# KanaLab/mesh

Measured on AMD Instinct MI355X. Metric: closest-point queries/sec vs 1M-face mesh at 1/2/4/8 MI355X + HBM GB/s, higher is better.
Workload: dtype f64; 1 GPU; C3: geodesic icosphere freq 224 (1003520 faces, 501762 vertices), 100000000 uniform queries in [-1.1,1.1]^3 (seed 3) per step, sharded contiguously over the GPUs; faces=1003520, queries_total=100000000, queries_per_gpu=100000000

## Files before the change

### mesh_amd/csrc/nearest.hip

```cpp
#include <algorithm>
#include <cstdlib>
#include <cstring>
#include <mutex>
#include <vector>
#include <type_traits>

#include "internal.h"


namespace msh {

struct DeferRec {
    uint32_t slot;
    uint32_t face;
    int32_t leaf;
    uint32_t roff;
    double best;
    uint32_t rcnt;
    uint32_t sbound;
};
static_assert(sizeof(DeferRec) == 32, "DeferRec must be 32 B");

#ifndef MSH_P2_SPLIT
#define MSH_P2_SPLIT 8
#endif
#ifndef MSH_P2_HEAVY
#define MSH_P2_HEAVY 0.97
#endif
constexpr unsigned kP2Split = MSH_P2_SPLIT;
constexpr double kP2Heavy = MSH_P2_HEAVY;
constexpr unsigned kP2SplitItems = 1u << 16;
constexpr uint32_t kP2Whole = 0xFFFFFFFFu;
struct P2Cand {
    double best;
    uint32_t face;
    int32_t leaf;
};

struct KnnArgs {
    const BNode* nodes;
    const void* leaves;
    size_t T;
    const double* q;
    const double* n;
    const uint32_t* perm;
    const uint32_t* qperm;
    uint32_t* inv_w;
    size_t S;
    QRes* res;
    double* res_w;
    uint32_t* out_face;
    uint32_t* out_part;
    double* out_pt;
    double* out_dist;
    double* out_w;
    double eps;
    double org[3];
    double tm;
    const double* orgs;
    size_t qper;
    size_t npm;
    size_t root0;
    unsigned* counters;
    unsigned ntiles;
    uint2* spill;
    int spill_depth;
    unsigned long long* stats;
    unsigned budget;
    int phase;
    bool direct;
    bool rec_leaf;
    bool list;
    const uint32_t* cut;
    int cut_wide;
    int cut_G;
    double cut_lo[3], cut_iw[3];
    size_t nunits;
    DeferRec* deferred;
    unsigned* n_deferred;
    unsigned max_deferred;
    uint2* resume;
    unsigned* n_resume;
    unsigned resume_cap;
// ... 151 lines not shown
            --sp;
            const Ent e = stack_get(lds, spill, sp);
            if (E::bound(e) <= pol.limf) {
                node = E::ref(e);
                return true;
            }
        }
        return false;
    }
    template <class Pol, bool STATS>
    __device__ inline bool step(const BNode* __restrict__ nodes, const QF& qf, Pol& pol, Ent* __restrict__ lds,
                                uint2* __restrict__ spill, unsigned& n_nodes, unsigned& n_leaves) {
        const NodeV nd = load_node(nodes, node);
        if (STATS) ++n_nodes;
        float d0, d1;
        node_child_bounds(nd, qf, d0, d1);
        const int c0 = nd.child(0), c1 = nd.child(1);
        bool h0 = d0 <= pol.limf, h1 = d1 <= pol.limf;
        if (h0 && c0 < 0) {
            pol.test(~c0);
            if (STATS) ++n_leaves;
            h0 = false;
        }
        if (h1 && c1 < 0) {
            pol.test(~c1);
            if (STATS) ++n_leaves;
            h1 = false;
        }
        h0 = h0 && d0 <= pol.limf;
        h1 = h1 && d1 <= pol.limf;
        if (h0 && h1) {
            int nearc = c0, farc = c1;
            float dfar = d1;
            if (d1 < d0) { nearc = c1; farc = c0; dfar = d0; }
            push((unsigned)farc, __float_as_uint(dfar), lds, spill);
            node = nearc;
            return true;
        }
        if (h0) { node = c0; return true; }
        if (h1) { node = c1; return true; }
        return pop(pol, lds, spill);
    }
    template <class Pol, bool STATS, bool PF = false>
    __device__ inline bool step_collect(const BNode* __restrict__ nodes, const QF& qf, const Pol& pol,
                                        Ent* __restrict__ lds, uint2* __restrict__ spill, unsigned& n_nodes, int& p0,
                                        int& p1, int room = 2, const float4* nb = nullptr, uint32_t wsl = 0) {
        bool more = false;
        if (node < 0) {
            p0 = ~node;
        } else {
            const NodeV nd = PF ? node_from_lds(nb) : load_node(nodes, node);
            if (STATS) ++n_nodes;
            float d0, d1;
            node_child_bounds(nd, qf, d0, d1);
            const int c0 = nd.child(0), c1 = nd.child(1);
            const float lim = pol.limf;
            const bool h0 = d0 <= lim, h1 = d1 <= lim;
            const bool l0 = h0 && c0 < 0, l1 = h1 && c1 < 0;
            const bool i0 = h0 && c0 >= 0, i1 = h1 && c1 >= 0;
            const bool first1 = d1 < d0;
            if (l0 && l1) {
                if (room < 2) {
                    p0 = first1 ? ~c1 : ~c0;
                    node = first1 ? c0 : c1;
                    more = true;
                } else {
                    p0 = ~c0;
                    p1 = ~c1;
                }
            } else {
                if (l0) p0 = ~c0;
                if (l1) p0 = ~c1;
                if (i0 && i1) push((unsigned)(first1 ? c0 : c1), __float_as_uint(first1 ? d0 : d1), lds, spill);
                if (i0 || i1) {
                    node = (i0 && i1) ? (first1 ? c1 : c0) : (i0 ? c0 : c1);
                    more = true;
                }
            }
        }
        const bool r = more || pop(pol, lds, spill);
        if (PF && r && node >= 0) node_prefetch(nodes, node, wsl);
        return r;
    }
};
typedef WalkerT<Ent8> Walker;

__device__ inline D3 heidrich_bary(const D3& p, const D3& a, const D3& b, const D3& c) {
    const D3 u = vsub(b, a), v = vsub(c, a);
    const D3 n = vcross(u, v);
    double s = n.x * n.x + n.y * n.y + n.z * n.z;
    if (s == 0.0) s = 2.220446049250313e-16;
    const double inv = 1.0 / s;
    const D3 w = vsub(p, a);
    const double b2 = vdot(vcross(u, w), n) * inv;
    const double b1 = vdot(vcross(w, v), n) * inv;
    return D3{1.0 - b1 - b2, b1, b2};
}

template <int MODE, class Pol>
__device__ inline void write_result(const KnnArgs& a, size_t i, const D3& q, const Pol& pol) {
    const bool rec = a.res && (!a.direct || a.phase == 1 || a.phase == 3 || a.phase == 4);
    const bool out = !a.res || a.direct;
    const size_t r = a.res ? (size_t)a.perm[i] : i;
    if constexpr (MODE == 2) {
        const double dist = pol.best_leaf >= 0 ? sqrt(pol.best) : NAN;
        if (rec) store_qres(a.res + i, pol.best_face, 0u, dist, 0.0, 0.0);
        if (out) {
            a.out_face[r] = pol.best_face;
            a.out_dist[r] = dist;
        }
        return;
    }
    const TriRec* tris = static_cast<const TriRec*>(a.leaves);
    D3 ta, tb, tc, o = D3{NAN, NAN, NAN}, w = D3{NAN, NAN, NAN};
    uint32_t face = MSH_NO_FACE;
    int part = 0;
    if (pol.best_leaf >= 0) {
        load_tri(tris, pol.best_leaf, ta, tb, tc, face);
        closest_on_triangle(q, ta, tb, tc, o, part);
        if (MODE == 3) w = heidrich_bary(o, ta, tb, tc);
    }
    if (rec) {
        store_qres(a.res + i, face, a.rec_leaf ? (uint32_t)pol.best_leaf : (uint32_t)part, o.x, o.y, o.z);
        if (MODE == 3 && !a.direct) {
            a.res_w[3 * i] = w.x;
            a.res_w[3 * i + 1] = w.y;
            a.res_w[3 * i + 2] = w.z;
        }
    }
    if (!out) return;
    a.out_face[r] = face;
    if (MODE == 0 && a.out_part) a.out_part[r] = (uint32_t)part;
    a.out_pt[3 * r] = o.x;
    a.out_pt[3 * r + 1] = o.y;
    a.out_pt[3 * r + 2] = o.z;
    if (MODE == 3) {
        a.out_w[3 * r] = w.x;
        a.out_w[3 * r + 1] = w.y;
        a.out_w[3 * r + 2] = w.z;
    }
}

template <int MODE>
struct PolOf { using T = TriPol; };
template <>
struct PolOf<1> { using T = NrmPol; };
template <>
struct PolOf<2> { using T = PtPol; };

template <int MODE>
__device__ inline typename PolOf<MODE>::T make_pol(const KnnArgs& a, size_t i, const D3& q) {
    typename PolOf<MODE>::T pol;
    if constexpr (MODE == 2) {
        pol.pts = static_cast<const PtRec*>(a.leaves);
    } else {
        pol.tris = static_cast<const TriRec*>(a.leaves);
    }
    pol.q = q;
    if constexpr (MODE == 1) {
        pol.qn = D3{a.n[3 * i], a.n[3 * i + 1], a.n[3 * i + 2]};
        const double nq = sqrt(vdot(pol.qn, pol.qn));
        pol.eps = a.eps;
        pol.pmin = fmin(a.eps * (1 - nq), a.eps * (1 + nq));
    }
    pol.best = INFINITY;
    pol.shared = INFINITY;
    pol.best_face = MSH_NO_FACE;
    pol.best_leaf = -1;
    pol.limf = INFINITY;
    return pol;
}


__device__ inline D3 load_q(const KnnArgs& a, size_t i) {
    const size_t r = a.qperm ? (size_t)a.qperm[i] : i;
    return D3{a.q[3 * r], a.q[3 * r + 1], a.q[3 * r + 2]};
}

#ifndef MSH_KLEAD
#define MSH_KLEAD 8
#endif
#ifndef MSH_KFWIN
#define MSH_KFWIN 64
#endif
#ifndef MSH_FOLLOW_CELL
#define MSH_FOLLOW_CELL 0
#endif
#ifndef MSH_RESUME
#define MSH_RESUME 1
#endif
constexpr unsigned kLead = MSH_KLEAD;
constexpr unsigned kLead2 = 256;
constexpr size_t kFWin = MSH_KFWIN;
constexpr size_t kLWin = 8;
static_assert(kLead2 % kLead == 0 && kLead2 / kLead >= 2, "kLead2: a multiple of kLead");
constexpr int kLeafQ = 4;
constexpr int kLeafRound = 2;

__device__ inline size_t slot_of(const KnnArgs& a, size_t k) {
    if (a.phase == 3) return k * kLead2;
    if (a.phase == 4) return k * kLead;
    if (a.phase == 1) {
        constexpr size_t r = kLead2 / kLead;
        return kLead * (k + k / (r - 1) + 1);
    }
    if (a.phase == 2) {
        const size_t g = k / (kLead - 1);
        return g * kLead + (k - g * (kLead - 1)) + 1;
    }
    return k;
}

__device__ inline int leader_leaf(const KnnArgs& a, size_t i, const D3& q, size_t window, size_t stride) {
    const size_t base = (i / window) * window;
    const size_t mesh = a.orgs ? i / a.qper : 0;
    double h = INFINITY;
    int leaf = -1;
    for (size_t L = 0; L < window; L += stride) {
        const size_t li = base + L;
        if (li >= a.S) break;
        if (a.orgs && li / a.qper != mesh) continue;
        const uint4 r0 = reinterpret_cast<const uint4*>(a.res + li)[0];
        if (r0.x == MSH_NO_FACE) continue;
        const double2 r1 = reinterpret_cast<const double2*>(a.res + li)[1];
        const double x = __longlong_as_double((long long)(((unsigned long long)r0.w << 32) | r0.z));
        const double dx = q.x - x, dy = q.y - r1.x, dz = q.z - r1.y;
        const double d2 = dx * dx + dy * dy + dz * dz;
        if (d2 < h) {
            h = d2;
            leaf = (int)r0.y;
        }
    }
    return leaf;
}

__device__ inline unsigned lanes_below(unsigned long long m) {
    return __builtin_amdgcn_mbcnt_hi((unsigned)(m >> 32), __builtin_amdgcn_mbcnt_lo((unsigned)m, 0u));
}

#ifndef MSH_KPEND
#define MSH_KPEND 32
#endif
constexpr int kPend = MSH_KPEND;
#ifndef MSH_TILE_PF
#define MSH_TILE_PF 1
#endif

constexpr unsigned kRing = 256;
constexpr size_t kListMaxLeaves = (size_t)1 << 26;
constexpr size_t kLeadMinLeaves = 4096;

#ifndef MSH_KNN_WAVES
#define MSH_KNN_WAVES 4
#endif
#define MSH_KNN_ATTR __attribute__((amdgpu_waves_per_eu(MODE == 1 ? 1 : MSH_KNN_WAVES)))
constexpr size_t kNoCell = ~(size_t)0;
__device__ inline size_t cut_cell(const KnnArgs& a, const D3& q) {
    if (!a.cut) return kNoCell;
    const double G = (double)a.cut_G;
    const double ux = (q.x - a.cut_lo[0]) * a.cut_iw[0], uy = (q.y - a.cut_lo[1]) * a.cut_iw[1],
                 uz = (q.z - a.cut_lo[2]) * a.cut_iw[2];
    if (!(ux >= 0.0 && ux < G && uy >= 0.0 && uy < G && uz >= 0.0 && uz < G)) return kNoCell;
    return ((size_t)(unsigned)uz * (size_t)a.cut_G + (unsigned)uy) * (size_t)a.cut_G + (unsigned)ux;
}
__device__ inline const uint32_t* cut_rec(const KnnArgs& a, size_t cell) {
    return a.cut + cell * (a.cut_wide ? 16 : 8);
}
template <class Pol, class W>
__device__ inline bool cut_start(const KnnArgs& a, size_t cell, const Pol& pol, W& w, typename W::Ent* __restrict__ lds,
                                 uint2* __restrict__ spill) {
    const uint32_t* r = cut_rec(a, cell);
    if (a.cut_wide) {
        const uint4* c = reinterpret_cast<const uint4*>(r);
        uint4 e[4];
#pragma unroll
        for (int j = 0; j < 4; ++j) e[j] = c[j];
        auto put = [&](uint32_t ref, uint32_t sb) {
            if (ref != kCutEmpty) w.push(ref, sb, lds, spill);
        };
#pragma unroll
        for (int j = 3; j >= 1; --j) {
            put(e[j].z, e[j].w);
            put(e[j].x, e[j].y);
        }
        put(e[0].z, e[0].w);
    } else {
        const uint4* c = reinterpret_cast<const uint4*>(r);
        const uint4 e0 = c[0], e1 = c[1];
        const uint32_t e[kCutK] = {e0.y, e0.z, e0.w, e1.x, e1.y, e1.z, e1.w};
#pragma unroll
        for (int j = kCutK - 1; j >= 0; --j)
            if ((int)e[j] >= 0) w.push((uint32_t)Ent4::ref(e[j]), e[j] & 0xFFE00000u, lds, spill);
    }
    return w.pop(pol, lds, spill);
}

template <int MODE, bool STATS, bool LIST, bool PF>
__global__ __launch_bounds__(kBlock) MSH_KNN_ATTR void k_knn(KnnArgs a) {
    constexpr bool kCompact = MODE == 0 || MODE == 3;
    constexpr bool kList = (MODE == 0 || MODE == 3) && LIST;
    constexpr bool kPF = kList && PF;
    typedef typename std::conditional<kPF, Ent4, Ent8>::type E;
    __shared__ typename E::T stk[kStack * kBlock];
    __shared__ float4 nbuf[kPF ? 4 * kBlock : 1];
    constexpr size_t kEntWords = kCompact && !kList ? (size_t)kBlock * kLeafQ * 2 : 1;
    constexpr size_t kListWords = kList ? 4 * (kRing + 64 * 4) : 1;
    __shared__ uint32_t lsh[kEntWords > kListWords ? kEntWords : kListWords];
    uint2* lent = reinterpret_cast<uint2*>(lsh);
    const int tid = threadIdx.x, lane = tid & 63;
    typename E::T* lds = stk + tid;
    const int wv_u = __builtin_amdgcn_readfirstlane(tid >> 6);
    const uint32_t wsl = (uint32_t)(size_t)(__attribute__((address_space(3))) float4*)(nbuf + (kPF ? wv_u * 256 : 0));
    const float4* nb = nbuf + (kPF ? (tid >> 6) * 256 + lane : 0);
    uint2* ent = lent + (kCompact ? (tid >> 6) * 64 * kLeafQ : 0);
    uint2* spill = a.spill ? a.spill + (size_t)blockIdx.x * kBlock * (size_t)a.spill_depth + tid : nullptr;
    const unsigned group = blockIdx.x & 7u;
    unsigned long long u_trav_it = 0, u_trav_lanes = 0, u_leaf_it = 0, u_leaf_lanes = 0;
    unsigned n_nodes = 0, n_leaves = 0;
    unsigned n_impr = 0, n_hinted = 0, n_hint_won = 0;
#if MSH_TILE_PF
    const unsigned glo = (unsigned)(((unsigned long long)a.ntiles * group) >> 3);
    const unsigned ghi = (unsigned)(((unsigned long long)a.ntiles * (group + 1)) >> 3);
    unsigned nxt = ~0u;
#endif
    for (;;) {
        unsigned tile = 0;
#if MSH_TILE_PF
        if (lane == 0) tile = (nxt != ~0u && glo + nxt < ghi) ? glo + nxt : dequeue_tile(a.counters, a.ntiles, group);
#else
        if (lane == 0) tile = dequeue_tile(a.counters, a.ntiles, group);
#endif
        tile = __shfl(tile, 0);
        if (tile >= a.ntiles) break;
        const size_t k = (size_t)tile * 64 + lane;
        size_t i = 0;
        bool live = k < a.nunits;
        if (live) {
            i = slot_of(a, k);
            live = i < a.S;
        }
        const D3 q = live ? load_q(a, i) : D3{0.0, 0.0, 0.0};
#if MSH_TILE_PF
        if (lane == 0) nxt = glo < ghi ? atomicAdd(&a.counters[group * 32], 1u) : ~0u;
#endif
        if (live && a.inv_w && !a.direct) a.inv_w[a.qperm[i]] = (uint32_t)i;
        auto pol = make_pol<MODE>(a, i, q);
        const bool fin = live && finite3(q);
        if (live && !fin) {
            if (!STATS || a.res) write_result<MODE>(a, i, q, pol);
        }
        int hint_leaf = -1;
        const size_t cell = kList && fin ? cut_cell(a, q) : kNoCell;
        if constexpr (MODE == 0 || MODE == 3) {
            if (kList && a.cut && cell != kNoCell && a.phase != 2) {
                const int lf = (int)cut_rec(a, cell)[0];
                if (STATS) hint_leaf = lf;
                if (lf >= 0) {
                    pol.test(lf);
                    if (STATS) {
                        ++n_leaves;
                        ++n_hinted;
                    }
                }
            } else if (fin && (a.phase == 2 || a.phase == 1)) {
                const int lf = a.phase == 2 ? leader_leaf(a, i, q, kFWin, kLead) : leader_leaf(a, i, q, kLWin * kLead2, kLead2);
                if (STATS) hint_leaf = lf;
#if MSH_FOLLOW_CELL
                const int lc = (kList && a.cut && cell != kNoCell) ? (int)cut_rec(a, cell)[0] : -1;
#pragma nounroll
                for (int j = 0; j < 2; ++j) {
                    const int h = j == 0 ? lf : (lc != lf ? lc : -1);
                    if (h >= 0) {
                        pol.test(h);
                        if (STATS) ++n_leaves;
                    }
                }
                if (STATS && lf >= 0) ++n_hinted;
#else
                if (lf >= 0) {
                    pol.test(lf);
                    if (STATS) {
                        ++n_leaves;
                        ++n_hinted;
                    }
                }
#endif
            }
        }
        if (a.T == 1) {
            if (fin) {
                pol.test(0);
                if (STATS) ++n_leaves;
                if (!STATS || a.res) write_result<MODE>(a, i, q, pol);
            }
            continue;
        }
        if constexpr (kList) {
          {
            QF qf;
            const int root = query_root(a, i, q, qf);
            WalkerT<E> w{root, 0};
            bool start = fin;
            if (cell != kNoCell) start = cut_start(a, cell, pol, w, lds, spill);
            if (kPF && start && w.node >= 0) node_prefetch(a.nodes, w.node, wsl);
            uint32_t* ring = lsh + (tid >> 6) * (kRing + 64 * 4);
            unsigned long long* bd = reinterpret_cast<unsigned long long*>(ring + kRing);
            unsigned long long* bfl = bd + 64;
            bool active = start, want_defer = false, deferred = false;
            int nq = 0;
            unsigned last_pos = 0;
            unsigned head = 0, tail = 0;
            unsigned steps = 0;
            const unsigned max_steps = (unsigned)min(a.T, (size_t)UINT_MAX);
            unsigned tot = 0;
            auto run_rounds = [&](unsigned upto) {
                while (head != upto) {
                    const unsigned n = min(64u, upto - head);
                    bd[lane] = (unsigned long long)__double_as_longlong(pol.best);
                    bfl[lane] = ~0ull;
                    const bool valid = (unsigned)lane < n;
                    const uint32_t en = ring[(head + (valid ? (unsigned)lane : 0u)) & (kRing - 1)];
                    const int src = (int)(en & 63u);
                    const int leaf = (int)(en >> 6);
                    const D3 x = D3{__shfl(pol.q.x, src), __shfl(pol.q.y, src), __shfl(pol.q.z, src)};
                    uint32_t f;
                    const double d2 = pol.eval(leaf, x, f);
                    const unsigned long long kb = (unsigned long long)__double_as_longlong(d2);
                    asm volatile("" ::: "memory");
                    if (valid) atomicMin(&bd[src], kb);
                    asm volatile("" ::: "memory");
                    if (valid && bd[src] == kb) atomicMin(&bfl[src], ((unsigned long long)f << 32) | (unsigned)leaf);
                    asm volatile("" ::: "memory");
                    const unsigned long long nb = bd[lane], nf = bfl[lane];
                    const double nd = __longlong_as_double((long long)nb);
                    const uint32_t nface = (uint32_t)(nf >> 32);
                    if (nf != ~0ull && (nd < pol.best || (nd == pol.best && nface < pol.best_face))) {
                        pol.best = nd;
                        pol.best_face = nface;
                        pol.best_leaf = (int)(uint32_t)nf;
                        pol.relim();
                        if (STATS) ++n_impr;
                    }
                    asm volatile("" ::: "memory");
                    if (STATS) {
                        if (valid) ++n_leaves;
                        if (lane == 0) {
                            ++u_leaf_it;
                            u_leaf_lanes += n;
                        }
                    }
                    head += n;
                }
                if ((int)(last_pos - head) < 0) nq = 0;
            };
            unsigned dslot = 0;
            for (;;) {
                if (want_defer && nq == 0) {
                    want_defer = false;
                    dslot = atomicAdd(a.n_deferred, 1u);
                    if (dslot < a.max_deferred) {
                        active = false;
                        deferred = true;
                    }
                }
                const bool can = active && !want_defer && nq < kPend;
                const bool any = __ballot(can) != 0ull;
                if (!any && tail == head) break;
                if (STATS) {
                    const int nt = __popcll(__ballot(can));
                    if (lane == 0 && any) {
                        ++u_trav_it;
                        u_trav_lanes += nt;
                    }
                }
                int l0 = -1, l1 = -1;
                if (can) {
                    active = w.template step_collect<decltype(pol), STATS, kPF>(a.nodes, qf, pol, lds, spill, n_nodes,
                                                                                  l0, l1, kPend - nq, nb, wsl);
                    ++steps;
                    if (STATS) ++tot;
                    if (active && steps >= max_steps) active = false;
                    if (active && steps == a.budget) want_defer = true;
                }
                if (l0 < 0) {
                    l0 = l1;
                    l1 = -1;
                }
                const unsigned long long m1 = __ballot(l0 >= 0), m2 = __ballot(l1 >= 0);
                const unsigned pos = tail + lanes_below(m1) + lanes_below(m2);
                if (l0 >= 0) {
                    ring[pos & (kRing - 1)] = ((uint32_t)l0 << 6) | (uint32_t)lane;
                    last_pos = pos;
                    ++nq;
                }
                if (l1 >= 0) {
                    ring[(pos + 1) & (kRing - 1)] = ((uint32_t)l1 << 6) | (uint32_t)lane;
                    last_pos = pos + 1;
                    ++nq;
                }
                tail += (unsigned)(__popcll(m1) + __popcll(m2));
                const unsigned upto = any ? head + ((tail - head) & ~63u) : tail;
                if (upto != head) run_rounds(upto);
            }
            if (deferred) {
                if ((a.phase == 1 || a.phase == 3 || a.phase == 4) && a.res) {
                    D3 o = D3{NAN, NAN, NAN};
                    uint32_t f = MSH_NO_FACE;
                    if (pol.best_leaf >= 0) {
                        D3 ta, tb, tc;
                        int part;
                        load_tri(static_cast<const TriRec*>(a.leaves), pol.best_leaf, ta, tb, tc, f);
                        closest_on_triangle(q, ta, tb, tc, o, part);
                    }
                    store_qres(a.res + i, f, (uint32_t)pol.best_leaf, o.x, o.y, o.z);
                }
                DeferRec r;
                r.slot = (uint32_t)i;
                r.face = pol.best_face;
                r.leaf = pol.best_leaf;
                r.roff = 0;
                r.best = pol.best;
                r.rcnt = 0;
                r.sbound = 0x7F800000u;
                if (a.max_best) atomicMax(a.max_best, (unsigned long long)__double_as_longlong(pol.best));
                if (a.resume) {
                    const unsigned cnt = (unsigned)w.sp + 1;
                    const unsigned off = atomicAdd(a.n_resume, cnt);
                    if (off + cnt <= a.resume_cap) {
                        uint2* dst = a.resume + off;
                        for (int j = 0; j < w.sp; ++j) {
                            const typename E::T e = stack_get(lds, spill, j);
                            dst[j] = make_uint2((uint32_t)E::ref(e), __float_as_uint(E::bound(e)));
                        }
                        dst[w.sp] = make_uint2((uint32_t)w.node, 0u);
                        r.roff = off;
                        r.rcnt = cnt;
                    }
                }
                a.deferred[dslot] = r;
            }
            if (STATS) {
                unsigned mx = tot, sm = tot;
                for (int o = 32; o > 0; o >>= 1) {
                    mx = max(mx, (unsigned)__shfl_xor((int)mx, o));
                    sm += (unsigned)__shfl_xor((int)sm, o);
                }
                unsigned long long* h = a.stats + 8 + 9 * (a.phase == 3 ? 0 : ((a.phase == 1 || a.phase == 4) ? 1 : 2));
                if (lane == 0) {
                    atomicAdd(h + 0, 1ull);
                    atomicAdd(h + 1, (unsigned long long)mx);
                    atomicAdd(h + 2, (unsigned long long)sm);
                    atomicAdd(h + 3, (unsigned long long)min(mx, 128u));
                    atomicAdd(h + 4, (unsigned long long)min(mx, 256u));
                    atomicAdd(h + 5, (unsigned long long)min(mx, 512u));
                }
                if (tot > 128) atomicAdd(h + 6, 1ull);
                if (tot > 256) atomicAdd(h + 7, 1ull);
                if (tot > 512) atomicAdd(h + 8, 1ull);
            }
            if (STATS && fin && hint_leaf >= 0 && pol.best_leaf == hint_leaf) ++n_hint_won;
            if (deferred) continue;
            if (fin && (!STATS || a.res)) write_result<MODE>(a, i, q, pol);
            continue;
          }
        }
        if constexpr (!kList) {
        {
            QF qf;
            const int root = query_root(a, i, q, qf);
            Walker w{root, 0};
            bool active = fin, deferred = false;
            int q0 = -1, q1 = -1, q2 = -1, q3 = -1, nq = 0;
            auto enqueue = [&](int x) {
                if (x < 0) return;
                if (kLeafQ > 3) q3 = q2;
                q2 = q1;
                q1 = q0;
                q0 = x;
                ++nq;
            };
            auto test_queue = [&](int most) {
                const int n = min(nq, most);
#pragma nounroll
                for (int k = 0; k < n; ++k) {
                    pol.test(q0);
                    q0 = q1;
                    q1 = q2;
                    if (kLeafQ > 3) q2 = q3;
                }
                nq -= n;
            };
            unsigned steps = 0;
            const unsigned max_steps = (unsigned)min(a.T, (size_t)UINT_MAX);
            unsigned tot = 0;
            for (;;) {
                const bool can = active && nq <= kLeafQ - 1;
                const bool has = nq > 0;
                const unsigned long long bl = __ballot(has);
                const unsigned long long bt = __ballot(can);
                if ((bl | bt) == 0ull) break;
                const bool flush = bt == 0ull || __ballot(has && !can) != 0ull;
                if (bl != 0ull && flush) {
                    if constexpr (kCompact) {
                        const unsigned long long lt = (1ull << lane) - 1ull;
                        const unsigned long long m1 = bl, m2 = __ballot(nq >= 2), m3 = __ballot(nq >= 3),
                                                 m4 = kLeafQ > 3 ? __ballot(nq >= 4) : 0ull;
                        const int pos = __popcll(m1 & lt) + __popcll(m2 & lt) + __popcll(m3 & lt) + __popcll(m4 & lt);
                        const int E = __popcll(m1) + __popcll(m2) + __popcll(m3) + __popcll(m4);
                        if (nq >= 1) ent[pos] = make_uint2((unsigned)q0, (unsigned)lane);
                        if (nq >= 2) ent[pos + 1] = make_uint2((unsigned)q1, (unsigned)lane);
                        if (nq >= 3) ent[pos + 2] = make_uint2((unsigned)q2, (unsigned)lane);
                        if (kLeafQ > 3 && nq >= 4) ent[pos + 3] = make_uint2((unsigned)q3, (unsigned)lane);
                        asm volatile("" ::: "memory");
                        bool better = false;
                        for (int base = 0; base < E; base += 64) {
                            const uint2 en = ent[min(base + lane, E - 1)];
                            const int src = (int)en.y;
                            const D3 x = D3{__shfl(pol.q.x, src), __shfl(pol.q.y, src), __shfl(pol.q.z, src)};
                            uint32_t f;
                            const double d2 = pol.eval((int)en.x, x, f);
                            if (STATS && base + lane < E) ++n_leaves;
#pragma unroll
                            for (int e = 0; e < kLeafQ; ++e) {
                                const int at = pos + e - base;
                                const bool mine = e < nq && at >= 0 && at < 64;
                                const int from = mine ? at : lane;
                                const double dk = __shfl(d2, from);
                                const uint32_t fk = (uint32_t)__shfl((int)f, from);
                                if (mine) {
                                    const bool b = pol.offer(dk, fk, e == 0 ? q0 : (e == 1 ? q1 : (e == 2 ? q2 : q3)));
                                    better |= b;
                                    if (STATS && b) ++n_impr;
                                }
                            }
                        }
                        asm volatile("" ::: "memory");
                        if (better) pol.relim();
                        if (STATS && lane == 0) {
                            u_leaf_it += (unsigned long long)((E + 63) / 64);
                            u_leaf_lanes += (unsigned long long)E;
                        }
                        nq = 0;
                    } else {
                        if (STATS && lane == 0) {
                            ++u_leaf_it;
// ... 365 lines not shown
__global__ __launch_bounds__(kBlock) void k_unpermute(const QRes* __restrict__ res, const double* __restrict__ w, int nw,
                                                      const uint32_t* __restrict__ inv, size_t S, SlotOut o) {
    const size_t j = (size_t)blockIdx.x * kBlock + threadIdx.x;
    if (j >= S) return;
    const size_t i = inv[j];
    const uint4 r0 = reinterpret_cast<const uint4*>(res + i)[0];
    const double2 r1 = reinterpret_cast<const double2*>(res + i)[1];
    const double x = __longlong_as_double((long long)(((unsigned long long)r0.w << 32) | r0.z));
    if (o.face) o.face[j] = r0.x;
    if (o.part) o.part[j] = r0.y;
    if (o.dist) o.dist[j] = x;
    if (o.pt) {
        o.pt[3 * j] = x;
        o.pt[3 * j + 1] = r1.x;
        o.pt[3 * j + 2] = r1.y;
    }
    for (int k = 0; k < nw; ++k) o.w[(size_t)nw * j + k] = w[(size_t)nw * i + k];
}

int unpermute_results(const QRes* d_res, const double* d_w, int nw, const uint32_t* d_inv, size_t S, const SlotOut& o,
                      hipStream_t s) {
    if (S == 0) return MSH_OK;
    TimedLaunch tl("unpermute", s);
    k_unpermute<<<(unsigned)((S + kBlock - 1) / kBlock), kBlock, 0, s>>>(d_res, d_w, nw, d_inv, S, o);
    MSH_HIP(hipGetLastError());
    return MSH_OK;
}

static int device_cus(int dev) {
    static std::mutex mu;
    static int cache[64] = {0};
    std::lock_guard<std::mutex> g(mu);
    if (dev < 0 || dev >= 64) return 256;
    if (!cache[dev]) {
        int n = 0;
        if (hipDeviceGetAttribute(&n, hipDeviceAttributeMultiprocessorCount, dev) != hipSuccess || n <= 0) n = 256;
        cache[dev] = n;
    }
    return cache[dev];
}

#ifndef MSH_BUDGET
#define MSH_BUDGET 512
#endif
constexpr unsigned kBudget = MSH_BUDGET;
constexpr unsigned kBudget3 = 256;
constexpr unsigned kBudget1 = MSH_BUDGET;
constexpr unsigned kKnnBlocksPerCU = 4;

template <int MODE, bool STATS>
static int launch_knn(msh_tree* tree, KnnArgs a, hipStream_t s, const char* timer) {
    if (a.S == 0) return MSH_OK;
    for (int k = 0; k < 3; ++k) a.org[k] = tree->origin[k];
    const unsigned ncu = (unsigned)device_cus(tree->device);
    Workspace& ws = tree->ws;
    MSH_TRY(ws.counters.reserve(13 * 32 * sizeof(unsigned)));
    a.counters = ws.counters.as<unsigned>();
    a.n_deferred = a.counters + 8 * 32;
    a.n_resume = a.counters + 10 * 32;
    MSH_HIP(hipMemsetAsync(a.counters, 0, 13 * 32 * sizeof(unsigned), s));
    const size_t n_lead = (a.S + kLead - 1) / kLead;
    const unsigned max_tiles = (unsigned)((a.S + 63) / 64);
    const unsigned nblk_max = std::min<unsigned>((max_tiles + 3) / 4, ncu * kKnnBlocksPerCU);
    const unsigned nblk2 = ncu * 2;
    const int need = tree->max_depth + 1 + 2 * kFront / 64 + 1 + (a.cut ? kCutK : 0);
    a.spill = nullptr;
    a.spill_depth = 0;
    if (need > kStack) {
        a.spill_depth = need - kStack + 1;
        MSH_TRY(ws.spill.reserve((size_t)std::max(nblk_max, nblk2) * kBlock * (size_t)a.spill_depth * sizeof(uint2)));
        a.spill = ws.spill.as<uint2>();
    }
    a.budget = kBudget;
    bool list_pf = false;
    {
        const char* e = getenv("MESH_AMD_LEAF_LIST");
        const int hook = e ? atoi(e) : 1;
        a.list = (MODE == 0 || MODE == 3) && hook != 0 && tree->B * tree->T < kListMaxLeaves;
        list_pf = a.list && hook != 2 && tree->B * tree->T <= kEnt4MaxLeaves;
    }
    const bool lead = kLead > 1 && (MODE == 0 || MODE == 3) && a.res != nullptr && a.S >= 64 * (size_t)kLead &&
                      a.T >= kLeadMinLeaves && !(a.list && a.cut);
    a.max_deferred = (unsigned)std::min<size_t>(a.S, (a.S / 16) + 65536);
    DevBuf& dbuf = ws.flags;
    MSH_TRY(dbuf.reserve((size_t)a.max_deferred * sizeof(DeferRec)));
    a.deferred = dbuf.as<DeferRec>();
    a.resume = nullptr;
    a.resume_cap = 0;
    a.cand = nullptr;
    a.heavy = nullptr;
    a.n_heavy = a.counters + 12 * 32;
    a.max_best = reinterpret_cast<unsigned long long*>(a.counters + 11 * 32);
    const unsigned split_cap = std::min<unsigned>(a.max_deferred, kP2SplitItems);
    if (kP2Split > 1 && (MODE == 0 || MODE == 3) && !STATS) {
        MSH_TRY(ws.p2cand.reserve((size_t)split_cap * (kP2Split * sizeof(P2Cand) + sizeof(unsigned))));
        a.cand = ws.p2cand.as<P2Cand>();
        a.heavy = reinterpret_cast<unsigned*>(a.cand + (size_t)split_cap * kP2Split);
    }
#if MSH_RESUME
    if (a.list) {
        const size_t cap = std::min<size_t>((size_t)1 << 26, std::max<size_t>((size_t)1 << 20, 48 * (a.S / 1024 + 1024)));
        MSH_TRY(ws.resume.reserve(cap * sizeof(uint2)));
        a.resume = ws.resume.as<uint2>();
        a.resume_cap = (unsigned)cap;
    }
#endif
    auto pass1 = [&](int phase, size_t nunits, const char* name) -> int {
        a.phase = phase;
        a.budget = phase == 3 ? kBudget3 : ((phase == 1 || phase == 4) ? kBudget1 : kBudget);
        a.budget = std::min<unsigned>(a.budget, (unsigned)std::max<size_t>(64, a.T / 16));
        a.nunits = nunits;
        a.ntiles = (unsigned)((nunits + 63) / 64);
        const unsigned nblk = std::min<unsigned>((a.ntiles + 3) / 4, ncu * kKnnBlocksPerCU);
        if (nblk == 0) return MSH_OK;
        TimedLaunch t1(name, s);
        if (a.list)
            if (list_pf)
                k_knn<MODE, STATS, (MODE == 0 || MODE == 3), (MODE == 0 || MODE == 3)><<<nblk, kBlock, 0, s>>>(a);
            else
                k_knn<MODE, STATS, (MODE == 0 || MODE == 3), false><<<nblk, kBlock, 0, s>>>(a);
        else
            k_knn<MODE, STATS, false, false><<<nblk, kBlock, 0, s>>>(a);
        MSH_HIP(hipGetLastError());
        return MSH_OK;
    };
    {
        TimedLaunch tl(timer, s);
        {
            TimedLaunch t1(STATS ? "knn_pass1_stats" : "knn_pass1", s);
            if (lead) {
                if (a.list && a.cut) {
                    MSH_TRY(pass1(4, n_lead, STATS ? "knn_lead_stats" : "knn_lead"));
                } else if (kLead2 > 0) {
                    constexpr size_t l2 = kLead2 ? kLead2 : 1;
                    const size_t n_super = (a.S + l2 - 1) / l2;
                    MSH_TRY(pass1(3, n_super, STATS ? "knn_lead2_stats" : "knn_lead2"));
                    MSH_HIP(hipMemsetAsync(a.counters, 0, 8 * 32 * sizeof(unsigned), s));
                    MSH_TRY(pass1(1, n_lead - n_super, STATS ? "knn_lead_stats" : "knn_lead"));
                } else {
                    MSH_TRY(pass1(1, n_lead, STATS ? "knn_lead_stats" : "knn_lead"));
                }
                MSH_HIP(hipMemsetAsync(a.counters, 0, 8 * 32 * sizeof(unsigned), s));
                MSH_TRY(pass1(2, a.S - n_lead, STATS ? "knn_follow_stats" : "knn_follow"));
            } else {
                MSH_TRY(pass1(0, a.S, STATS ? "knn_all_stats" : "knn_all"));
            }
        }
        {
            TimedLaunch t2(STATS ? "knn_pass2_stats" : "knn_pass2", s);
            if (a.cand) {
                k_p2_plan<<<64, kBlock, 0, s>>>(a);
                MSH_HIP(hipGetLastError());
            }
            k_knn_coop<MODE, STATS><<<nblk2, kBlock, 0, s>>>(a);
            MSH_HIP(hipGetLastError());
            if (a.cand) {
                k_knn_combine<MODE><<<(split_cap + kBlock - 1) / kBlock, kBlock, 0, s>>>(a);
                MSH_HIP(hipGetLastError());
            }
        }
        if (STATS && getenv("MESH_AMD_P2_DUMP")) {
            unsigned nd = 0;
            MSH_HIP(hipMemcpyAsync(&nd, a.n_deferred, sizeof(unsigned), hipMemcpyDeviceToHost, s));
            MSH_HIP(hipStreamSynchronize(s));
            nd = std::min(nd, a.max_deferred);
            std::vector<DeferRec> h(nd);
            if (nd) MSH_HIP(hipMemcpy(h.data(), a.deferred, nd * sizeof(DeferRec), hipMemcpyDeviceToHost));
            if (FILE* f = fopen(getenv("MESH_AMD_P2_DUMP"), "wb")) {
                fwrite(h.data(), sizeof(DeferRec), nd, f);
                fclose(f);
            }
        }
    }
    return MSH_OK;
}


template <int MODE, bool STATS>
static int run_knn(msh_tree* tree, KnnArgs a, const QueryOrder& ord, const SlotOut& o, int nw, hipStream_t s,
                   const char* timer) {
    if (a.S == 0) return MSH_OK;
    a.q = ord.q;
    a.perm = ord.perm;
    if (!ord.gathered) {
        a.qperm = ord.perm;
        a.inv_w = const_cast<uint32_t*>(ord.inv);
    }
    Workspace& ws = tree->ws;
    if (ord.perm) {
        MSH_TRY(ws.res.reserve(a.S * sizeof(QRes)));
        a.res = ws.res.as<QRes>();
        a.direct = !STATS && (MODE == 0 || MODE == 3);
        a.rec_leaf = a.direct || STATS;
        if (nw && !a.direct) {
            MSH_TRY(ws.res_w.reserve(a.S * (size_t)nw * sizeof(double)));
            a.res_w = ws.res_w.as<double>();
        }
        if (a.direct) {
            a.out_face = o.face;
// ... 336 lines not shown
```

Baseline: 2.572 billion queries/s.

## Add lean specialized list-path kNN kernel for direct cut-grid phase-0 queries

Measured after the change: 2.641 billion queries/s (median of 6 runs). 2.7% higher.

```diff
diff --git a/mesh_amd/csrc/nearest.hip b/mesh_amd/csrc/nearest.hip
--- a/mesh_amd/csrc/nearest.hip
+++ b/mesh_amd/csrc/nearest.hip
@@ -1,4 +1,5 @@
 #include <algorithm>
+#include <cstddef>
 #include <cstdlib>
 #include <cstring>
 #include <mutex>
@@ -316,6 +317,56 @@
         if (PF && r && node >= 0) node_prefetch(nodes, node, wsl);
         return r;
     }
+    template <class Pol, class SpillOf>
+    __device__ inline bool step_list(const BNode* __restrict__ nodes, const QF& qf, const Pol& pol, Ent* __restrict__ lds,
+                                     SpillOf&& spill_of, int& p0, int& p1, const float4* nb, uint32_t wsl) {
+        const bool deep = __ballot(sp >= kStack) != 0ull;
+        bool more = false;
+        if (node < 0) {
+            p0 = ~node;
+        } else {
+            const NodeV nd = node_from_lds(nb);
+            float d0, d1;
+            node_child_bounds(nd, qf, d0, d1);
+            const int c0 = nd.child(0), c1 = nd.child(1);
+            const float lim = pol.limf;
+            const bool h0 = d0 <= lim, h1 = d1 <= lim;
+            const bool l0 = h0 && c0 < 0, l1 = h1 && c1 < 0;
+            const bool i0 = h0 && c0 >= 0, i1 = h1 && c1 >= 0;
+            const bool first1 = d1 < d0;
+            if (l0) p0 = ~c0;
+            if (l1) p1 = ~c1;
+            if (i0 && i1) {
+                const Ent e = E::make((unsigned)(first1 ? c0 : c1), __float_as_uint(first1 ? d0 : d1));
+                if (!deep)
+                    lds[sp * kBlock] = e;
+                else
+                    stack_put(lds, spill_of(), sp, e);
+                ++sp;
+            }
+            if (i0 || i1) {
+                node = (i0 && i1) ? (first1 ? c1 : c0) : (i0 ? c0 : c1);
+                more = true;
+            }
+        }
+        if (!more) {
+            if (!deep) {
+                while (sp > 0) {
+                    --sp;
+                    const Ent e = lds[sp * kBlock];
+                    if (E::bound(e) <= pol.limf) {
+                        node = E::ref(e);
+                        more = true;
+                        break;
+                    }
+                }
+            } else {
+                more = pop(pol, lds, spill_of());
+            }
+        }
+        if (more && node >= 0) node_prefetch(nodes, node, wsl);
+        return more;
+    }
 };
 typedef WalkerT<Ent8> Walker;
 
@@ -374,6 +425,48 @@
         a.out_w[3 * r + 2] = w.z;
     }
 }
+
+template <int MODE, class Pol>
+__device__ inline void write_direct(const TriRec* __restrict__ tris, size_t r, const D3& q, const Pol& pol,
+                                    uint32_t* out_face, uint32_t* out_part, double* out_pt, double* out_w) {
+    D3 ta, tb, tc, o = D3{NAN, NAN, NAN}, w = D3{NAN, NAN, NAN};
+    uint32_t face = MSH_NO_FACE;
+    int part = 0;
+    if (pol.best_leaf >= 0) {
+        load_tri(tris, pol.best_leaf, ta, tb, tc, face);
+        closest_on_triangle(q, ta, tb, tc, o, part);
+        if (MODE == 3) w = heidrich_bary(o, ta, tb, tc);
+    }
+    out_face[r] = face;
+    if (MODE == 0 && out_part) out_part[r] = (uint32_t)part;
+    out_pt[3 * r] = o.x;
+    out_pt[3 * r + 1] = o.y;
+    out_pt[3 * r + 2] = o.z;
+    if (MODE == 3) {
+        out_w[3 * r] = w.x;
+        out_w[3 * r + 1] = w.y;
+        out_w[3 * r + 2] = w.z;
+    }
+}
+
+static_assert(std::is_standard_layout<KnnArgs>::value && std::is_trivially_copyable<KnnArgs>::value &&
+                  alignof(KnnArgs) <= 8,
+              "cold_arg reads KnnArgs fields at their offsetof from the start of the kernarg segment");
+template <class T>
+__device__ inline T cold_arg(size_t off) {
+    typedef __attribute__((address_space(4))) const char* KP;
+    KP p = (KP)__builtin_amdgcn_kernarg_segment_ptr();
+    asm volatile("" : "+s"(p));
+    return *(__attribute__((address_space(4))) const T*)(p + off);
+}
+#ifndef MSH_LEAN_COLD
+#define MSH_LEAN_COLD 1
+#endif
+#if MSH_LEAN_COLD
+#define MSH_COLD_ARG(f) cold_arg<decltype(KnnArgs::f)>(offsetof(KnnArgs, f))
+#else
+#define MSH_COLD_ARG(f) (a.f)
+#endif
 
 template <int MODE>
 struct PolOf { using T = TriPol; };
@@ -480,6 +573,19 @@
 #define MSH_TILE_PF 1
 #endif
 
+#ifndef MSH_KNN_LEAN
+#define MSH_KNN_LEAN 1
+#endif
+#ifndef MSH_LIST_RESERVE
+#define MSH_LIST_RESERVE 0
+#endif
+#ifndef MSH_LEAN_STEP
+#define MSH_LEAN_STEP 1
+#endif
+#ifndef MSH_LEAN_STATE
+#define MSH_LEAN_STATE 1
+#endif
+
 constexpr unsigned kRing = 256;
 constexpr size_t kListMaxLeaves = (size_t)1 << 26;
 constexpr size_t kLeadMinLeaves = 4096;
@@ -528,12 +634,39 @@
     }
     return w.pop(pol, lds, spill);
 }
-
-template <int MODE, bool STATS, bool LIST, bool PF>
+static_assert(kCutK <= kStack, "a cut record's entries fit the LDS stack");
+template <class Pol, class W>
+__device__ inline bool cut_start_narrow(const uint32_t* __restrict__ cut, size_t cell, const Pol& pol, W& w,
+                                        uint32_t* __restrict__ lds) {
+    const uint4* c = reinterpret_cast<const uint4*>(cut + cell * 8);
+    const uint4 e0 = c[0], e1 = c[1];
+    const uint32_t e[kCutK] = {e0.y, e0.z, e0.w, e1.x, e1.y, e1.z, e1.w};
+#pragma unroll
+    for (int j = kCutK - 1; j >= 0; --j)
+        if ((int)e[j] >= 0) {
+            lds[w.sp * kBlock] = Ent4::make((uint32_t)Ent4::ref(e[j]), e[j] & 0xFFE00000u);
+            ++w.sp;
+        }
+    while (w.sp > 0) {
+        --w.sp;
+        const uint32_t t = lds[w.sp * kBlock];
+        if (Ent4::bound(t) <= pol.limf) {
+            w.node = Ent4::ref(t);
+            return true;
+        }
+    }
+    return false;
+}
+
+template <int MODE, bool STATS, bool LIST, bool PF, bool LEAN = false>
 __global__ __launch_bounds__(kBlock) MSH_KNN_ATTR void k_knn(KnnArgs a) {
     constexpr bool kCompact = MODE == 0 || MODE == 3;
     constexpr bool kList = (MODE == 0 || MODE == 3) && LIST;
     constexpr bool kPF = kList && PF;
+    constexpr bool kLean = LEAN;
+    constexpr bool kLeanStep = LEAN && MSH_LEAN_STEP;
+    constexpr bool kLeanState = LEAN && MSH_LEAN_STATE;
+    static_assert(!LEAN || (kPF && !STATS), "the lean kernel is a list-path, prefetching, uninstrumented one");
     typedef typename std::conditional<kPF, Ent4, Ent8>::type E;
     __shared__ typename E::T stk[kStack * kBlock];
     __shared__ float4 nbuf[kPF ? 4 * kBlock : 1];
@@ -547,7 +680,7 @@
     const uint32_t wsl = (uint32_t)(size_t)(__attribute__((address_space(3))) float4*)(nbuf + (kPF ? wv_u * 256 : 0));
     const float4* nb = nbuf + (kPF ? (tid >> 6) * 256 + lane : 0);
     uint2* ent = lent + (kCompact ? (tid >> 6) * 64 * kLeafQ : 0);
-    uint2* spill = a.spill ? a.spill + (size_t)blockIdx.x * kBlock * (size_t)a.spill_depth + tid : nullptr;
+    uint2* spill = (!kLeanStep && a.spill) ? a.spill + (size_t)blockIdx.x * kBlock * (size_t)a.spill_depth + tid : nullptr;
     const unsigned group = blockIdx.x & 7u;
     unsigned long long u_trav_it = 0, u_trav_lanes = 0, u_leaf_it = 0, u_leaf_lanes = 0;
     unsigned n_nodes = 0, n_leaves = 0;
@@ -568,24 +701,39 @@
         if (tile >= a.ntiles) break;
         const size_t k = (size_t)tile * 64 + lane;
         size_t i = 0;
-        bool live = k < a.nunits;
+        bool live = k < (kLean ? a.S : a.nunits);
         if (live) {
-            i = slot_of(a, k);
+            i = kLean ? k : slot_of(a, k);
             live = i < a.S;
         }
         const D3 q = live ? load_q(a, i) : D3{0.0, 0.0, 0.0};
 #if MSH_TILE_PF
         if (lane == 0) nxt = glo < ghi ? atomicAdd(&a.counters[group * 32], 1u) : ~0u;
 #endif
-        if (live && a.inv_w && !a.direct) a.inv_w[a.qperm[i]] = (uint32_t)i;
+        if constexpr (!kLean)
+            if (live && a.inv_w && !a.direct) a.inv_w[a.qperm[i]] = (uint32_t)i;
         auto pol = make_pol<MODE>(a, i, q);
         const bool fin = live && finite3(q);
+        auto lean_write = [&]() {
+            if constexpr (kLean)
+                write_direct<MODE>(static_cast<const TriRec*>(a.leaves), (size_t)MSH_COLD_ARG(perm)[i], q, pol,
+                                   MSH_COLD_ARG(out_face), MSH_COLD_ARG(out_part), MSH_COLD_ARG(out_pt),
+                                   MSH_COLD_ARG(out_w));
+        };
         if (live && !fin) {
-            if (!STATS || a.res) write_result<MODE>(a, i, q, pol);
+            if constexpr (kLean)
+                lean_write();
+            else if (!STATS || a.res)
+                write_result<MODE>(a, i, q, pol);
         }
         int hint_leaf = -1;
         const size_t cell = kList && fin ? cut_cell(a, q) : kNoCell;
-        if constexpr (MODE == 0 || MODE == 3) {
+        if constexpr (kLean) {
+            if (cell != kNoCell) {
+                const int lf = (int)a.cut[cell * 8];
+                if (lf >= 0) pol.test(lf);
+            }
+        } else if constexpr (MODE == 0 || MODE == 3) {
             if (kList && a.cut && cell != kNoCell && a.phase != 2) {
                 const int lf = (int)cut_rec(a, cell)[0];
                 if (STATS) hint_leaf = lf;
@@ -621,7 +769,7 @@
 #endif
             }
         }
-        if (a.T == 1) {
+        if (!kLean && a.T == 1) {
             if (fin) {
                 pol.test(0);
                 if (STATS) ++n_leaves;
@@ -632,20 +780,37 @@
         if constexpr (kList) {
           {
             QF qf;
-            const int root = query_root(a, i, q, qf);
+            int root = 0;
+            if constexpr (kLean) {
+                const double o[3] = {a.org[0], a.org[1], a.org[2]};
+                qf = make_qf(q, o, a.tm);
+            } else {
+                root = query_root(a, i, q, qf);
+            }
             WalkerT<E> w{root, 0};
             bool start = fin;
-            if (cell != kNoCell) start = cut_start(a, cell, pol, w, lds, spill);
+            if constexpr (kLeanStep) {
+                if (cell != kNoCell) start = cut_start_narrow(a.cut, cell, pol, w, lds);
+            } else {
+                if (cell != kNoCell) start = cut_start(a, cell, pol, w, lds, spill);
+            }
+            auto lean_spill = [&]() -> uint2* {
+                return MSH_COLD_ARG(spill) + (size_t)blockIdx.x * kBlock * (size_t)MSH_COLD_ARG(spill_depth) + tid;
+            };
             if (kPF && start && w.node >= 0) node_prefetch(a.nodes, w.node, wsl);
             uint32_t* ring = lsh + (tid >> 6) * (kRing + 64 * 4);
             unsigned long long* bd = reinterpret_cast<unsigned long long*>(ring + kRing);
             unsigned long long* bfl = bd + 64;
             bool active = start, want_defer = false, deferred = false;
+            enum { kIdle = 0, kWalk = 1, kPast = 2, kDeferred = 3 };
+            int st = start ? kWalk : kIdle;
             int nq = 0;
             unsigned last_pos = 0;
             unsigned head = 0, tail = 0;
             unsigned steps = 0;
             const unsigned max_steps = (unsigned)min(a.T, (size_t)UINT_MAX);
+            unsigned budget = a.budget;
+            if constexpr (kLean) asm volatile("" : "+s"(budget));
             unsigned tot = 0;
             auto run_rounds = [&](unsigned upto) {
                 while (head != upto) {
@@ -687,17 +852,26 @@
                 }
                 if ((int)(last_pos - head) < 0) nq = 0;
             };
-            unsigned dslot = 0;
+            unsigned dslot = ~0u;
+          lean_again:
             for (;;) {
-                if (want_defer && nq == 0) {
+                if constexpr (kLeanState) {
+                    if (st == kPast && nq == 0) st = kDeferred;
+                } else if (want_defer && nq == 0) {
                     want_defer = false;
-                    dslot = atomicAdd(a.n_deferred, 1u);
-                    if (dslot < a.max_deferred) {
+                    if constexpr (kLean) {
                         active = false;
                         deferred = true;
+                    } else {
+                        dslot = atomicAdd(a.n_deferred, 1u);
+                        if (dslot < a.max_deferred) {
+                            active = false;
+                            deferred = true;
+                        }
                     }
                 }
-                const bool can = active && !want_defer && nq < kPend;
+                const bool can = (kLeanState ? st == kWalk : active && !want_defer) &&
+                                 nq < ((kLeanStep || MSH_LIST_RESERVE) ? kPend - 1 : kPend);
                 const bool any = __ballot(can) != 0ull;
                 if (!any && tail == head) break;
                 if (STATS) {
@@ -709,12 +883,19 @@
                 }
                 int l0 = -1, l1 = -1;
                 if (can) {
-                    active = w.template step_collect<decltype(pol), STATS, kPF>(a.nodes, qf, pol, lds, spill, n_nodes,
-                                                                                  l0, l1, kPend - nq, nb, wsl);
+                    if constexpr (kLeanStep)
+                        active = w.step_list(a.nodes, qf, pol, lds, lean_spill, l0, l1, nb, wsl);
+                    else
+                        active = w.template step_collect<decltype(pol), STATS, kPF>(a.nodes, qf, pol, lds, spill,
+                                                                                      n_nodes, l0, l1, kPend - nq, nb,
+                                                                                      wsl);
                     ++steps;
                     if (STATS) ++tot;
                     if (active && steps >= max_steps) active = false;
-                    if (active && steps == a.budget) want_defer = true;
+                    if constexpr (kLeanState)
+                        st = !active ? kIdle : (steps == budget ? kPast : kWalk);
+                    else if (active && steps == budget)
+                        want_defer = true;
                 }
                 if (l0 < 0) {
                     l0 = l1;
@@ -736,7 +917,53 @@
                 const unsigned upto = any ? head + ((tail - head) & ~63u) : tail;
                 if (upto != head) run_rounds(upto);
             }
-            if (deferred) {
+            if constexpr (kLean) {
+                bool again = false;
+                const unsigned max_deferred = MSH_COLD_ARG(max_deferred);
+                if constexpr (kLeanState) deferred = st == kDeferred;
+                if (deferred && dslot == ~0u) {
+                    dslot = atomicAdd(MSH_COLD_ARG(n_deferred), 1u);
+                    if (dslot >= max_deferred) {
+                        deferred = false;
+                        active = true;
+                        st = kWalk;
+                        again = true;
+                    }
+                }
+                if (__ballot(again) != 0ull) goto lean_again;
+                deferred = deferred && dslot < max_deferred;
+            }
+            if constexpr (kLean) {
+              if (deferred) {
+                DeferRec r;
+                r.slot = (uint32_t)i;
+                r.face = pol.best_face;
+                r.leaf = pol.best_leaf;
+                r.roff = 0;
+                r.best = pol.best;
+                r.rcnt = 0;
+                r.sbound = 0x7F800000u;
+                unsigned long long* const max_best = MSH_COLD_ARG(max_best);
+                if (max_best) atomicMax(max_best, (unsigned long long)__double_as_longlong(pol.best));
+                uint2* const resume = MSH_COLD_ARG(resume);
+                if (resume) {
+                    const unsigned cnt = (unsigned)w.sp + 1;
+                    const unsigned off = atomicAdd(MSH_COLD_ARG(n_resume), cnt);
+                    if (off + cnt <= MSH_COLD_ARG(resume_cap)) {
+                        uint2* dst = resume + off;
+                        const uint2* sp_col = w.sp > kStack ? lean_spill() : nullptr;
+                        for (int j = 0; j < w.sp; ++j) {
+                            const typename E::T e = stack_get(lds, sp_col, j);
+                            dst[j] = make_uint2((uint32_t)E::ref(e), __float_as_uint(E::bound(e)));
+                        }
+                        dst[w.sp] = make_uint2((uint32_t)w.node, 0u);
+                        r.roff = off;
+                        r.rcnt = cnt;
+                    }
+                }
+                MSH_COLD_ARG(deferred)[dslot] = r;
+              }
+            } else if (deferred) {
                 if ((a.phase == 1 || a.phase == 3 || a.phase == 4) && a.res) {
                     D3 o = D3{NAN, NAN, NAN};
                     uint32_t f = MSH_NO_FACE;
@@ -794,7 +1021,11 @@
             }
             if (STATS && fin && hint_leaf >= 0 && pol.best_leaf == hint_leaf) ++n_hint_won;
             if (deferred) continue;
-            if (fin && (!STATS || a.res)) write_result<MODE>(a, i, q, pol);
+            if constexpr (kLean) {
+                if (fin) lean_write();
+            } else {
+                if (fin && (!STATS || a.res)) write_result<MODE>(a, i, q, pol);
+            }
             continue;
           }
         }
@@ -1326,6 +1557,8 @@
     const bool lead = kLead > 1 && (MODE == 0 || MODE == 3) && a.res != nullptr && a.S >= 64 * (size_t)kLead &&
                       a.T >= kLeadMinLeaves && !(a.list && a.cut);
     a.max_deferred = (unsigned)std::min<size_t>(a.S, (a.S / 16) + 65536);
+    if (const char* e = getenv("MESH_AMD_MAX_DEFERRED"))
+        a.max_deferred = std::min<unsigned>(a.max_deferred, (unsigned)std::max(1, atoi(e)));
     DevBuf& dbuf = ws.flags;
     MSH_TRY(dbuf.reserve((size_t)a.max_deferred * sizeof(DeferRec)));
     a.deferred = dbuf.as<DeferRec>();
@@ -1349,6 +1582,12 @@
         a.resume_cap = (unsigned)cap;
     }
 #endif
+    bool lean = false;
+    if constexpr (MSH_KNN_LEAN && !STATS && (MODE == 0 || MODE == 3)) {
+        const char* e = getenv("MESH_AMD_KNN_LEAN");
+        lean = (!e || atoi(e) != 0) && a.list && list_pf && a.cut && !a.cut_wide && a.direct && a.T > 1 &&
+               !a.orgs;
+    }
     auto pass1 = [&](int phase, size_t nunits, const char* name) -> int {
         a.phase = phase;
         a.budget = phase == 3 ? kBudget3 : ((phase == 1 || phase == 4) ? kBudget1 : kBudget);
@@ -1357,8 +1596,12 @@
         a.ntiles = (unsigned)((nunits + 63) / 64);
         const unsigned nblk = std::min<unsigned>((a.ntiles + 3) / 4, ncu * kKnnBlocksPerCU);
         if (nblk == 0) return MSH_OK;
-        TimedLaunch t1(name, s);
-        if (a.list)
+        const bool take_lean = lean && phase == 0;
+        TimedLaunch t1(take_lean ? "knn_lean" : name, s);
+        constexpr bool kCanLean = MSH_KNN_LEAN && !STATS && (MODE == 0 || MODE == 3);
+        if (take_lean) {
+            if constexpr (kCanLean) k_knn<MODE, false, true, true, true><<<nblk, kBlock, 0, s>>>(a);
+        } else if (a.list)
             if (list_pf)
                 k_knn<MODE, STATS, (MODE == 0 || MODE == 3), (MODE == 0 || MODE == 3)><<<nblk, kBlock, 0, s>>>(a);
             else
```
